# jmoraispk/DeepMIMO

Measured on AMD Instinct MI355X. Metric: user-channels/sec, higher is better.
Workload: dtype f16x3-split MFMA, f32 accumulate

## Files before the change

### deepmimo_amd/csrc/k2c_beam_power.hip

```cpp
#include "k2_mfma_frag.h"
#include "dmx_tuning.h"
#include <stdlib.h>

namespace dmx {

static constexpr int BP_SLOT = 16 * 1024;
static constexpr int BP_BUFS = 2;

struct BeamPowArgs {
    int64_t user_begin;
    int m_rx, ue_mh, n_beams;
    int M;
    int K;
    const int32_t* sc;
    double inv_n;
    const float2* ftab;
    const int32_t* fexp;
    float* out;
    int32_t* best;
    int adaptive;
};

__host__ __device__ inline size_t beam_pow_lds_bytes(int M, int NW) {
    const size_t nblk = ((size_t)M + 32 * NW - 1) / (32 * NW);
    return (size_t)BP_BUFS * (NW / 4) * BP_SLOT + LPAD * (8 + 4 + 4) + 16 + nblk * NW * 32 * 4;
}

template <int NW>
__global__ __launch_bounds__(NW * 64, 4) void k2c_beam_power(WsView ws, BeamPowArgs a, int64_t user_count) {
    constexpr int BP_WAVES = NW, BP_CHUNK = NW / 4, MAX_ROWS = 32 * NW;
    extern __shared__ __attribute__((aligned(16))) unsigned char smem[];
    unsigned char* bbuf = smem;
    float* bbuf_f = reinterpret_cast<float*>(smem);
    float2* qtab = reinterpret_cast<float2*>(smem + (size_t)BP_BUFS * BP_CHUNK * BP_SLOT);
    float* crtab = reinterpret_cast<float*>(qtab + LPAD);
    float* citab = crtab + LPAD;
    float* misc = citab + LPAD;
    float* rs = misc + 4;
    const int tid = threadIdx.x, lane = tid & 63;
    const int wave = __builtin_amdgcn_readfirstlane(tid >> 6);
    const int col = lane & 31, hh = lane >> 5;
    const int B = a.n_beams, M = a.M, P = ws.P;
    const int nwide = (a.K + 31) >> 5;
    const int nblk = (M + MAX_ROWS - 1) / MAX_ROWS;

    for (int64_t ul = blockIdx.x; ul < user_count; ul += gridDim.x) {
        const int64_t u = a.user_begin + ul;
        int n_act = ws.n_keep[u];
        n_act = n_act < LPAD ? n_act : LPAD;
        if (n_act == 0) {
            for (int b = tid; b < B; b += BP_WAVES * 64) a.out[(size_t)ul * B + b] = 0.f;
            if (a.best && tid == 0) a.best[ul] = -1;
            continue;
        }
        const size_t rb = (size_t)u * P;
        if (wave == 0) {
            float m = 0.f;
            if (lane < n_act) m = fmaxf(fabsf(ws.c_re[rb + lane]), fabsf(ws.c_im[rb + lane]));
            for (int off = 32; off > 0; off >>= 1) m = fmaxf(m, __shfl_xor(m, off));
            const int l0w = ((n_act - 1) >> 3) << 3;
            float a2 = 0.f;
            if (lane < n_act) a2 = fmaf(ws.c_re[rb + lane], ws.c_re[rb + lane], ws.c_im[rb + lane] * ws.c_im[rb + lane]);
            float m2 = a2, mw2 = lane >= l0w ? a2 : 0.f;
            for (int off = 32; off > 0; off >>= 1) { m2 = fmaxf(m2, __shfl_xor(m2, off)); mw2 = fmaxf(mw2, __shfl_xor(mw2, off)); }
            if (lane == 0) misc[3] = (a.adaptive && l0w >= 8 && mw2 * 4194304.0f <= m2) ? 1.f : 0.f;
            int e;
            (void)frexpf(m, &e);
            const float gs = ldexpf(1.0f, 10 - e);
            if (lane < LPAD) {
                const bool ok = lane < n_act;
                const double q = ok ? (double)ws.dn[rb + lane] * a.inv_n : 0.0;
                const double qh = rint(q * 4096.0) * (1.0 / 4096.0);
                qtab[lane] = make_float2((float)qh, (float)(q - qh));
                crtab[lane] = ok ? ws.c_re[rb + lane] * gs : 0.f;
                citab[lane] = ok ? ws.c_im[rb + lane] * gs : 0.f;
            }
            const int ea = 6 - a.fexp[ul];
            if (lane == 0) { misc[0] = ldexpf(1.0f, e - 10 - ea); misc[1] = ldexpf(1.0f, ea); misc[2] = gs; }
        }
        __syncthreads();
        const float ascale = misc[1];
        const int nfull = ((n_act + 7) >> 3) - (misc[3] != 0.f ? 1 : 0);

        for (int blk = 0; blk < nblk; ++blk) {
            const int row0 = blk * MAX_ROWS;
            const int nrows = (M - row0) < MAX_ROWS ? (M - row0) : MAX_ROWS;
            const int ntiles = (nrows + 31) >> 5;
            const int ntp = ntiles <= 1 ? 1 : (ntiles <= 2 ? 2 : (ntiles <= 4 ? 4 : 8));
            const int tile = wave & (ntp - 1), grp = wave / ntp, ngrp = BP_WAVES / ntp;
            const bool active = tile < ntiles;
            h8 Ah[4], Al[4];
#pragma unroll
            for (int s = 0; s < 4; ++s) { Ah[s] = h8{0, 0, 0, 0, 0, 0, 0, 0}; Al[s] = Ah[s]; }
            if (active) {
                const int r = row0 + (tile << 5) + col;
                const bool pok = r < M;
                const int rx = pok ? r / B : 0, bm = pok ? r - rx * B : 0;
                const double yr = (double)(rx % a.ue_mh), zr = (double)(rx / a.ue_mh);
                const float2* frow = a.ftab + ((size_t)ul * B + bm) * P;
#pragma unroll
                for (int s = 0; s < 4; ++s) {
                    if (8 * s < n_act) {
#pragma unroll
                        for (int jj = 0; jj < 4; ++jj) {
                            const int pl = 8 * s + 4 * hh + jj;
                            h2 vh = {(_Float16)0.f, (_Float16)0.f}, vl = vh;
                            if (pok && pl < n_act) {
                                float sn, cs;
                                sincos_rev(frac_rev(yr * ws.rx_y[rb + pl] + zr * ws.rx_z[rb + pl]), sn, cs);
                                const float2 f = frow[pl];
                                split2_f16((cs * f.x - sn * f.y) * ascale, (cs * f.y + sn * f.x) * ascale, vh, vl, ws.neg_one);
                            }
                            Ah[s][2 * jj] = vh[0]; Ah[s][2 * jj + 1] = vh[1];
                            Al[s][2 * jj] = vl[0]; Al[s][2 * jj + 1] = vl[1];
                        }
                    }
                }
            }
            typedef float pv2 __attribute__((ext_vector_type(2)));
            pv2 rowsum[8];
#pragma unroll
            for (int i = 0; i < 8; ++i) rowsum[i] = pv2{0.f, 0.f};

            auto generate = [&](int c0, int buf) {
                const int wsi = c0 + (wave >> 2), st = wave & 3;
                const int kidx = (wsi << 5) + col;
                const bool kok = wsi < nwide && kidx < a.K;
                const int kki = kok ? a.sc[kidx] : 0;
                const float kl = (float)(kki & 4095), kf = (float)kki;
                h8* slot = reinterpret_cast<h8*>(bbuf + (size_t)(buf * BP_CHUNK + (wave >> 2)) * BP_SLOT);
                h8 rh = h8{0, 0, 0, 0, 0, 0, 0, 0}, rl = rh, ih = rh, il = rh;
                if (kok && 8 * st < n_act) {
#pragma unroll
                    for (int jj = 0; jj < 4; ++jj) {
                        const int pl = 8 * st + 4 * hh + jj;
                        const float2 q = qtab[pl];
                        const float p1 = q.x * kl;
                        float sn, cs;
                        sincos_rev(fmaf(q.y, kf, p1 - rintf(p1)), sn, cs);
                        const float cr = crtab[pl], ci = citab[pl];
                        h2 vh, vl;
                        split2_f16(cr * cs + ci * sn, ci * cs - cr * sn, vh, vl, ws.neg_one);
                        const unsigned hb = __builtin_bit_cast(unsigned, vh), lb = __builtin_bit_cast(unsigned, vl);
                        const h2 reh = __builtin_bit_cast(h2, hb ^ 0x80000000u), rel = __builtin_bit_cast(h2, lb ^ 0x80000000u);
                        const h2 imh = __builtin_bit_cast(h2, __builtin_amdgcn_alignbit(hb, hb, 16));
                        const h2 iml = __builtin_bit_cast(h2, __builtin_amdgcn_alignbit(lb, lb, 16));
                        rh[2 * jj] = reh[0]; rh[2 * jj + 1] = reh[1]; rl[2 * jj] = rel[0]; rl[2 * jj + 1] = rel[1];
                        ih[2 * jj] = imh[0]; ih[2 * jj + 1] = imh[1]; il[2 * jj] = iml[0]; il[2 * jj + 1] = iml[1];
                    }
                }
                slot[(4 * st + 0) * 64 + lane] = rh;
                slot[(4 * st + 1) * 64 + lane] = rl;
                slot[(4 * st + 2) * 64 + lane] = ih;
                slot[(4 * st + 3) * 64 + lane] = il;
            };
            __syncthreads();
            generate(0, 0);
            __syncthreads();
            int buf = 0;
            for (int c0 = 0; c0 < nwide; c0 += BP_CHUNK, buf ^= 1) {
                if (c0 + BP_CHUNK < nwide) generate(c0 + BP_CHUNK, buf ^ 1);
                if (active) {
                    for (int j = grp; j < BP_CHUNK && c0 + j < nwide; j += ngrp) {
                        const h8* slot = reinterpret_cast<const h8*>(bbuf + (size_t)(buf * BP_CHUNK + j) * BP_SLOT);
                        f16v are, aim;
#pragma unroll
                        for (int i = 0; i < 16; ++i) { are[i] = 0.f; aim[i] = 0.f; }
#pragma unroll
                        for (int s = 0; s < 4; ++s) {
                            if (8 * s < n_act) {
                                const h8 rh = slot[(4 * s + 0) * 64 + lane], rl = slot[(4 * s + 1) * 64 + lane];
                                const h8 ih = slot[(4 * s + 2) * 64 + lane], il = slot[(4 * s + 3) * 64 + lane];
                                are = __builtin_amdgcn_mfma_f32_32x32x16_f16(Ah[s], rh, are, 0, 0, 0);
                                aim = __builtin_amdgcn_mfma_f32_32x32x16_f16(Ah[s], ih, aim, 0, 0, 0);
                                if (s >= nfull) continue;
                                are = __builtin_amdgcn_mfma_f32_32x32x16_f16(Ah[s], rl, are, 0, 0, 0);
                                aim = __builtin_amdgcn_mfma_f32_32x32x16_f16(Ah[s], il, aim, 0, 0, 0);
                                are = __builtin_amdgcn_mfma_f32_32x32x16_f16(Al[s], rh, are, 0, 0, 0);
                                aim = __builtin_amdgcn_mfma_f32_32x32x16_f16(Al[s], ih, aim, 0, 0, 0);
                            }
                        }
                        DMX_MFMA_RESULT_GUARD2(are, aim);
#pragma unroll
                        for (int i = 0; i < 8; ++i) {
                            const pv2 re = {are[2 * i], are[2 * i + 1]}, im = {aim[2 * i], aim[2 * i + 1]};
                            const pv2 p = __builtin_elementwise_fma(re, re, im * im);
                            rowsum[i] += pv2{__builtin_amdgcn_sqrtf(p.x), __builtin_amdgcn_sqrtf(p.y)};
                        }
                    }
                }
                __syncthreads();
            }
            if (active) {
#pragma unroll
                for (int i = 0; i < 16; ++i) {
                    float v = (i & 1) ? rowsum[i >> 1].y : rowsum[i >> 1].x;
                    for (int off = 16; off > 0; off >>= 1) v += __shfl_xor(v, off);
                    if (col == 0) rs[((blk * BP_WAVES + wave) << 5) + (i & 3) + 8 * (i >> 2) + 4 * hh] = v;
                }
            }
        }
        __syncthreads();
        const float norm = misc[0] / ((float)a.m_rx * (float)a.K);
        for (int b = tid; b < B; b += BP_WAVES * 64) {
            float t = 0.f;
            for (int rx = 0; rx < a.m_rx; ++rx) {
                const int r = rx * B + b, blk = r / MAX_ROWS, w = r - blk * MAX_ROWS, tile = w >> 5;
                const int nrows = (M - blk * MAX_ROWS) < MAX_ROWS ? (M - blk * MAX_ROWS) : MAX_ROWS;
                const int ntiles = (nrows + 31) >> 5;
                const int ntp = ntiles <= 1 ? 1 : (ntiles <= 2 ? 2 : (ntiles <= 4 ? 4 : 8));
                for (int g = 0; g < BP_WAVES / ntp; ++g) t += rs[((blk * BP_WAVES + g * ntp + tile) << 5) + (w & 31)];
            }
            t *= norm;
            a.out[(size_t)ul * B + b] = t;
            bbuf_f[b] = t;
        }
        __syncthreads();
        if (a.best && tid == 0) {
            int arg = 0;
            float mx = bbuf_f[0];
            for (int b = 1; b < B; ++b) { if (bbuf_f[b] > mx) { mx = bbuf_f[b]; arg = b; } }
            a.best[ul] = arg;
        }
        __syncthreads();
    }
}

int launch_beam_project(const dmx_params& prm, const WsView& ws, int64_t user_begin, int64_t user_count,
                        const float2* codebook, int n_beams, void* beam_ws, hipStream_t stream, BeamTabs* tabs);

int launch_beam_power(const dmx_params& prm, const WsView& ws, int64_t user_begin, int64_t user_count,
                      const float2* codebook, int n_beams, void* beam_ws, float* out_amp, int32_t* out_best, hipStream_t stream) {
    if (user_count == 0 || n_beams == 0) return DMX_OK;
    BeamTabs t;
    int rc = launch_beam_project(prm, ws, user_begin, user_count, codebook, n_beams, beam_ws, stream, &t);
    if (rc) return rc;
    BeamPowArgs a;
    a.user_begin = user_begin;
    a.m_rx = prm.ue_shape[0] * prm.ue_shape[1];
    a.ue_mh = prm.ue_shape[0];
    a.n_beams = n_beams;
    a.M = a.m_rx * n_beams;
    a.K = prm.n_selected;
    a.sc = prm.selected_subcarriers;
    a.inv_n = 1.0 / (double)prm.n_subcarriers;
    a.ftab = t.ftab;
    a.fexp = t.fexp;
    a.out = out_amp;
    a.best = out_best;
    a.adaptive = (prm.flags & DMX_FLAG_ADAPTIVE_TERMS) ? 1 : 0;
    const int nw = tuning_int("DMX_BEAM_WAVES", 8) == 4 ? 4 : 8;
    const size_t smem = beam_pow_lds_bytes(a.M, nw);
    if (smem > 160 * 1024) { set_error("%d x %d (rx, beam) rows are too many for the beam-power kernel", a.m_rx, n_beams); return DMX_ERR_SHAPE; }
    const void* kfn = nw == 4 ? reinterpret_cast<const void*>(k2c_beam_power<4>) : reinterpret_cast<const void*>(k2c_beam_power<8>);
    hipError_t e = hipFuncSetAttribute(kfn, hipFuncAttributeMaxDynamicSharedMemorySize, (int)smem);
    if (e != hipSuccess) { set_error("hipFuncSetAttribute failed: %s", hipGetErrorString(e)); return DMX_ERR_LAUNCH; }
    int per_cu = 0;
    if (hipOccupancyMaxActiveBlocksPerMultiprocessor(&per_cu, kfn, nw * 64, smem) != hipSuccess || per_cu < 1) {
        (void)hipGetLastError();
        per_cu = 1;
    }
    int64_t grid = (int64_t)device_cu_count() * per_cu;
    const int64_t g4 = user_count / 4;
    if (g4 > grid) grid = g4 < 4 * grid ? g4 : 4 * grid;
    if (grid > user_count) grid = user_count;
    if (nw == 4) hipLaunchKernelGGL(k2c_beam_power<4>, dim3((unsigned)grid), dim3(256), smem, stream, ws, a, user_count);
    else hipLaunchKernelGGL(k2c_beam_power<8>, dim3((unsigned)grid), dim3(512), smem, stream, ws, a, user_count);
    e = hipGetLastError();
    if (e != hipSuccess) { set_error("k2c_beam_power launch failed: %s", hipGetErrorString(e)); return DMX_ERR_LAUNCH; }
    return DMX_OK;
}

}
```

Baseline: 6.505 million.

## Pack sparse tail k-step hi/lo split terms into a single MFMA pair

When the last 8-path K-step holds at most two active paths, the A and B fragments are rearranged. The hi and lo split parts of those paths go into otherwise-empty K slots of one MFMA operand, so the tail needs one re/im MFMA pair instead of three. Low-part LDS loads move after the nfull check so skipped steps no longer read them, and n_act and the weak flag are made wave-uniform with readfirstlane. The cost is extra shuffles and a special-case generate path, and the packed layout has to map exactly onto the MFMA K lanes to stay correct.

```diff
diff --git a/deepmimo_amd/csrc/k2c_beam_power.hip b/deepmimo_amd/csrc/k2c_beam_power.hip
--- a/deepmimo_amd/csrc/k2c_beam_power.hip
+++ b/deepmimo_amd/csrc/k2c_beam_power.hip
@@ -47,7 +47,7 @@
     for (int64_t ul = blockIdx.x; ul < user_count; ul += gridDim.x) {
         const int64_t u = a.user_begin + ul;
         int n_act = ws.n_keep[u];
-        n_act = n_act < LPAD ? n_act : LPAD;
+        n_act = __builtin_amdgcn_readfirstlane(n_act < LPAD ? n_act : LPAD);
         if (n_act == 0) {
             for (int b = tid; b < B; b += BP_WAVES * 64) a.out[(size_t)ul * B + b] = 0.f;
             if (a.best && tid == 0) a.best[ul] = -1;
@@ -80,7 +80,10 @@
         }
         __syncthreads();
         const float ascale = misc[1];
-        const int nfull = ((n_act + 7) >> 3) - (misc[3] != 0.f ? 1 : 0);
+        const int tail = (n_act - 1) >> 3;
+        const bool pack = n_act - 8 * tail <= 2;
+        const bool weak = __builtin_amdgcn_readfirstlane(__float_as_int(misc[3])) != 0;
+        const int nfull = tail + ((pack || weak) ? 0 : 1);
 
         for (int blk = 0; blk < nblk; ++blk) {
             const int row0 = blk * MAX_ROWS;
@@ -89,6 +92,7 @@
             const int ntp = ntiles <= 1 ? 1 : (ntiles <= 2 ? 2 : (ntiles <= 4 ? 4 : 8));
             const int tile = wave & (ntp - 1), grp = wave / ntp, ngrp = BP_WAVES / ntp;
             const bool active = tile < ntiles;
+            typedef unsigned u4v __attribute__((ext_vector_type(4)));
             h8 Ah[4], Al[4];
 #pragma unroll
             for (int s = 0; s < 4; ++s) { Ah[s] = h8{0, 0, 0, 0, 0, 0, 0, 0}; Al[s] = Ah[s]; }
@@ -116,6 +120,14 @@
                         }
                     }
                 }
+#pragma unroll
+                for (int s = 0; s < 4; ++s) {
+                    if (pack && s == tail) {
+                        const u4v h = __builtin_bit_cast(u4v, Ah[s]), l = __builtin_bit_cast(u4v, Al[s]);
+                        const unsigned l0 = __shfl(l[0], col), l1 = __shfl(l[1], col);
+                        Ah[s] = __builtin_bit_cast(h8, hh ? u4v{l0, l1, 0u, 0u} : u4v{h[0], h[1], h[0], h[1]});
+                    }
+                }
             }
             typedef float pv2 __attribute__((ext_vector_type(2)));
             pv2 rowsum[8];
@@ -128,25 +140,40 @@
                 const bool kok = wsi < nwide && kidx < a.K;
                 const int kki = kok ? a.sc[kidx] : 0;
                 const float kl = (float)(kki & 4095), kf = (float)kki;
-                h8* slot = reinterpret_cast<h8*>(bbuf + (size_t)(buf * BP_CHUNK + (wave >> 2)) * BP_SLOT);
-                h8 rh = h8{0, 0, 0, 0, 0, 0, 0, 0}, rl = rh, ih = rh, il = rh;
+                u4v* slot = reinterpret_cast<u4v*>(bbuf + (size_t)(buf * BP_CHUNK + (wave >> 2)) * BP_SLOT);
+                auto gsplit = [&](int pl, unsigned& hb, unsigned& lb) {
+                    const float2 q = qtab[pl];
+                    const float p1 = q.x * kl;
+                    float sn, cs;
+                    sincos_rev(fmaf(q.y, kf, p1 - rintf(p1)), sn, cs);
+                    const float cr = crtab[pl], ci = citab[pl];
+                    h2 vh, vl;
+                    split2_f16(cr * cs + ci * sn, ci * cs - cr * sn, vh, vl, ws.neg_one);
+                    hb = __builtin_bit_cast(unsigned, vh); lb = __builtin_bit_cast(unsigned, vl);
+                };
+                auto re_of = [](unsigned w) { return w ^ 0x80000000u; };
+                auto im_of = [](unsigned w) { return __builtin_amdgcn_alignbit(w, w, 16); };
+                u4v rh = u4v{0, 0, 0, 0}, rl = rh, ih = rh, il = rh;
+                const bool pk = pack && st == tail;
+                if (pk) {
+                    if (kok) {
+                        unsigned h0, l0, h1, l1;
+                        gsplit(8 * st, h0, l0);
+                        gsplit(8 * st + 1, h1, l1);
+                        rh = u4v{re_of(h0), re_of(h1), hh ? 0u : re_of(l0), hh ? 0u : re_of(l1)};
+                        ih = u4v{im_of(h0), im_of(h1), hh ? 0u : im_of(l0), hh ? 0u : im_of(l1)};
+                    }
+                    slot[(4 * st + 0) * 64 + lane] = rh;
+                    slot[(4 * st + 2) * 64 + lane] = ih;
+                    return;
+                }
                 if (kok && 8 * st < n_act) {
 #pragma unroll
                     for (int jj = 0; jj < 4; ++jj) {
-                        const int pl = 8 * st + 4 * hh + jj;
-                        const float2 q = qtab[pl];
-                        const float p1 = q.x * kl;
-                        float sn, cs;
-                        sincos_rev(fmaf(q.y, kf, p1 - rintf(p1)), sn, cs);
-                        const float cr = crtab[pl], ci = citab[pl];
-                        h2 vh, vl;
-                        split2_f16(cr * cs + ci * sn, ci * cs - cr * sn, vh, vl, ws.neg_one);
-                        const unsigned hb = __builtin_bit_cast(unsigned, vh), lb = __builtin_bit_cast(unsigned, vl);
-                        const h2 reh = __builtin_bit_cast(h2, hb ^ 0x80000000u), rel = __builtin_bit_cast(h2, lb ^ 0x80000000u);
-                        const h2 imh = __builtin_bit_cast(h2, __builtin_amdgcn_alignbit(hb, hb, 16));
-                        const h2 iml = __builtin_bit_cast(h2, __builtin_amdgcn_alignbit(lb, lb, 16));
-                        rh[2 * jj] = reh[0]; rh[2 * jj + 1] = reh[1]; rl[2 * jj] = rel[0]; rl[2 * jj + 1] = rel[1];
-                        ih[2 * jj] = imh[0]; ih[2 * jj + 1] = imh[1]; il[2 * jj] = iml[0]; il[2 * jj + 1] = iml[1];
+                        unsigned hb, lb;
+                        gsplit(8 * st + 4 * hh + jj, hb, lb);
+                        rh[jj] = re_of(hb); rl[jj] = re_of(lb);
+                        ih[jj] = im_of(hb); il[jj] = im_of(lb);
                     }
                 }
                 slot[(4 * st + 0) * 64 + lane] = rh;
@@ -169,11 +196,11 @@
 #pragma unroll
                         for (int s = 0; s < 4; ++s) {
                             if (8 * s < n_act) {
-                                const h8 rh = slot[(4 * s + 0) * 64 + lane], rl = slot[(4 * s + 1) * 64 + lane];
-                                const h8 ih = slot[(4 * s + 2) * 64 + lane], il = slot[(4 * s + 3) * 64 + lane];
+                                const h8 rh = slot[(4 * s + 0) * 64 + lane], ih = slot[(4 * s + 2) * 64 + lane];
                                 are = __builtin_amdgcn_mfma_f32_32x32x16_f16(Ah[s], rh, are, 0, 0, 0);
                                 aim = __builtin_amdgcn_mfma_f32_32x32x16_f16(Ah[s], ih, aim, 0, 0, 0);
                                 if (s >= nfull) continue;
+                                const h8 rl = slot[(4 * s + 1) * 64 + lane], il = slot[(4 * s + 3) * 64 + lane];
                                 are = __builtin_amdgcn_mfma_f32_32x32x16_f16(Ah[s], rl, are, 0, 0, 0);
                                 aim = __builtin_amdgcn_mfma_f32_32x32x16_f16(Ah[s], il, aim, 0, 0, 0);
                                 are = __builtin_amdgcn_mfma_f32_32x32x16_f16(Al[s], rh, are, 0, 0, 0);
```

Result: no change. 6.507 million, median of 5 (+0.0%).
